# harvardinformatics/IMCoalHMM

Measured on AMD Instinct MI355X. Metric: alignment columns/sec (forward pass), 20-state isolation HMM, higher is better.
Workload: dtype f64

## Files before the change

imcoalhmm_amd/csrc/imcoal_fwd.hip:

```cpp
#include <hip/hip_runtime.h>

#include <algorithm>
#include <array>
#include <cerrno>
#include <climits>
#include <cmath>
#include <cstdint>
#include <cstdio>
#include <cstdlib>
#include <cstring>
#include <list>
#include <atomic>
#include <chrono>
#include <map>
#include <set>
#include <memory>
#include <mutex>
#include <condition_variable>
#include <string>
#include <vector>

#include <sys/stat.h>
#include <unistd.h>

// ... 885 lines not shown
            if (int rc = alloc_symbols(o)) return rc;
            if (int rc = ingest_pump(lk, st, payload, slab, &slabs, fill, [&](int b, uint64_t off, uint64_t len) -> int {
                    const uint32_t columns = (uint32_t)std::min<uint64_t>(4 * len, L - 4 * off);
                    HIP_TRY(hipMemcpyAsync(st.dev[b].get(), st.host[b], (size_t)len, hipMemcpyHostToDevice, g.stream));
                    hipLaunchKernelGGL(k_ing_unpack2, dim3((uint32_t)((len + ING_THREADS - 1) / ING_THREADS)), dim3(ING_THREADS), 0, g.stream,
                                       (const uint8_t *)st.dev[b].get(), columns, o->d_sym + 4 * off * unit, o->wide_raw ? 1 : 0);
                    return IMC_OK;
                }))
                return rc;
            st.release();
            return validate_device_symbols(o->d_sym, (int)unit, (size_t)L, nsym, ">= nsym");
        }
        HIP_TRY(raw.alloc((size_t)payload));
        if (int rc = ingest_pump(lk, st, payload, slab, &slabs, fill, [&](int b, uint64_t off, uint64_t len) -> int {
                HIP_TRY(hipMemcpyAsync(raw.get() + off, st.host[b], (size_t)len, hipMemcpyHostToDevice, g.stream));
                return IMC_OK;
            }))
            return rc;
        st.release();
        const int rc = adopt_device_symbols(o, raw.get(), (int)(h.bits / 8), ">= nsym");
        raw.reset();
        return rc;
    };
    int rc = work();
    if (rc == IMC_OK) rc = finish_device_chunk(lk, o);
    if (rc == IMC_OK) note_ingest(2, payload, slabs, L);
    return ingest_result(rc, o, out);
}

int obs_from_file_device(const char *path, int nsym, imc_obs **out, bool *declined)
{
    FILE *fp = std::fopen(path, "rb");
    if (!fp) return fail(IMC_ERR_IO, std::string("cannot open ") + path + ": " + std::strerror(errno));
    struct Closer { FILE *f; ~Closer() { std::fclose(f); } } closer{fp};
    struct stat sb;
    if (fstat(fileno(fp), &sb) != 0 || !S_ISREG(sb.st_mode)) { *declined = true; return IMC_OK; }
    char head[8];
    const size_t nh = std::fread(head, 1, 8, fp);
    const bool cache = nh == 8 && std::memcmp(head, imc::kCacheMagic, 8) == 0;
    imc::CacheHeader h;
    if (cache) {
        const imc::IoResult hr = imc::read_cache_header(fp, path, nsym, h);
        if (hr.code) return fail(hr.code, hr.msg);
        if (h.bits == 16 && nsym <= imc::kByteAlphabet) { *declined = true; return IMC_OK; }
        if (h.L >= (uint64_t)1 << 31) return fail(IMC_ERR_ARG, "chunk too long (limit 2^31-1 columns per chunk)");
    } else
        std::rewind(fp);
    std::unique_lock<std::mutex> lk(g_mu);
    if (int rc = ensure_ctx()) return rc;
    HIP_TRY(hipSetDevice(g.device));
    return cache ? ingest_cache(lk, fp, h, path, nsym, out) : ingest_text(lk, fp, (uint64_t)sb.st_size, path, nsym, out, declined);
}

int obs_from_pairwise(const char *seq1, const char *seq2, size_t L, imc_obs **out)
{
    std::unique_lock<std::mutex> lk(g_mu);
    if (int rc = ensure_ctx()) return rc;
    HIP_TRY(hipSetDevice(g.device));
    const size_t columns = std::min<size_t>(ingest_slab_bytes() / 2, std::max<size_t>(L, imc::kMinSlabBytes / 2)), half = (columns + 15) & ~(size_t)15;
    IngestStage st;
    if (int rc = st.alloc(2 * half, L > half ? 2 : 1)) return rc;
    imc_obs *o = obs_new(L, 3);
    if (!o) return fail(IMC_ERR_OOM, "host allocation failed");
    uint64_t slabs = 0;
    int rc = alloc_symbols(o);
    if (rc == IMC_OK)
        rc = ingest_pump(lk, st, L, half, &slabs,
                         [&](int b, uint64_t off, uint64_t len) -> int {
                             std::memcpy(st.host[b], seq1 + off, (size_t)len);
                             std::memcpy(st.host[b] + half, seq2 + off, (size_t)len);
                             return IMC_OK;
                         },
                         [&](int b, uint64_t off, uint64_t len) -> int {
                             HIP_TRY(hipMemcpyAsync(st.dev[b].get(), st.host[b], half + (size_t)len, hipMemcpyHostToDevice, g.stream));
                             hipLaunchKernelGGL(k_ing_pairwise, dim3((uint32_t)((len + 4 * ING_THREADS - 1) / (4 * ING_THREADS))), dim3(ING_THREADS), 0, g.stream,
                                                (const uint8_t *)st.dev[b].get(), (const uint8_t *)st.dev[b].get() + half, (uint32_t)len, o->d_sym + off);
                             return IMC_OK;
                         });
    st.release();
    if (rc == IMC_OK) rc = finish_device_chunk(lk, o);
    if (rc == IMC_OK) note_ingest(3, 2 * (uint64_t)L, slabs, L);
    return ingest_result(rc, o, out);
}

int token_level(const imc_obs *obs, int alphabet_limit)
{
    int level = -1;
    if (obs->dict)
        for (int l = 0; l < imc::kNumLevels; ++l)
            if (obs->alphabet[l] <= alphabet_limit && obs->alphabet[l] > obs->nsym && obs->d_tok[l]) level = l;
    return level;
}

int recompress_alphabet(int nsym, std::vector<imc_obs *> &obs, bool on_device)
{
    std::sort(obs.begin(), obs.end(), [](const imc_obs *x, const imc_obs *y) { return x->id < y->id; });
    obs.erase(std::unique(obs.begin(), obs.end()), obs.end());
    const bool wide_raw = nsym > imc::kByteAlphabet;
    const size_t unit = wide_raw ? sizeof(imc::tok_t) : 1;
    PhaseTimer tm;
    size_t total = 0;
    for (imc_obs *o : obs) total += o->L;
    if (total < imc::TrainLimits().train_min) return IMC_OK;
    const size_t share = imc::recompress_share(obs.size(), wide_raw);
    std::vector<std::vector<uint8_t>> raw(obs.size());
    {
        std::lock_guard<std::mutex> lk(g_mu);
        bool same = obs[0]->dict != nullptr;
        for (imc_obs *o : obs) same = same && o->dict == obs[0]->dict;
        if (same && obs[0]->dict->trained_on >= total) return IMC_OK;
        HIP_TRY(hipSetDevice(g.device));
        for (size_t k = 0; k < obs.size(); ++k) {
            raw[k].resize((on_device ? std::min(obs[k]->L, share) : obs[k]->L) * unit);
            HIP_TRY(hipMemcpy(raw[k].data(), obs[k]->d_sym, raw[k].size(), hipMemcpyDeviceToHost));
        }
    }
    std::vector<uint8_t> sample = imc::recompress_sample(raw, share, unit);
    tm.mark();
    const std::shared_ptr<DictDev> nd = make_dictionary(symbols_in(sample, wide_raw), nsym, total);
    std::vector<uint8_t>().swap(sample);
    tm.mark();
    std::vector<imc::EncodedLevels> enc(obs.size());
    const bool zipped = nd->dict.alphabet > nsym;
    if (zipped && !on_device)
        for (size_t k = 0; k < obs.size(); ++k) {
            const HostSymbols sym = symbols_in(raw[k], wide_raw);
            imc::encode_levels(nd->dict, sym.bytes, sym.wide, obs[k]->L, enc[k]);
            std::vector<uint8_t>().swap(raw[k]);
        }
    tm.mark();
    std::unique_lock<std::mutex> lk(g_mu);
    wait_all_idle(lk);
    HIP_TRY(hipSetDevice(g.device));
    HIP_TRY(hipDeviceSynchronize());
    drop_plans_using(obs.data(), obs.size());
    if (!zipped) return IMC_OK;
    if (int rc = publish_dictionary(nsym, nd)) return rc;
    if (on_device) {
        for (imc_obs *o : obs) release_tokens(o);
        if (int rc = device_encode(nd, obs.data(), obs.size())) return rc;
    } else
        for (size_t k = 0; k < obs.size(); ++k) {
            release_tokens(obs[k]);
            if (int rc = install_encoding(obs[k], nd, enc[k])) return rc;
        }
    tm.mark();
    if (PhaseTimer::enabled())
        std::fprintf(stderr, "[imc host] recompress %zu chunks, %zu columns: copy back %.1f ms, train %.1f ms, encode %.1f ms, install %.1f ms (%s encoder)\n",
                     obs.size(), total, tm.ms(0), tm.ms(1), tm.ms(2), tm.ms(3), on_device ? "device" : "host");
    return IMC_OK;
}


using ChainFn = void (*)(const ChainDesc *, int, const uint32_t *, uint32_t, uint32_t, const double *, const int *,
                         const int *, uint32_t, double *, int *, double *, int);

struct KernelChoice : imc::KernelFacts {
    void (*plain)(PropArgs) = nullptr;
    void (*zip)(PropArgs) = nullptr;
    ChainFn chain = nullptr;
    void (*big_table_raw)(BigArgs) = nullptr;
    void (*big_table_level)(BigArgs, const uint16_t *, int) = nullptr;
    void (*big_prop)(BigArgs, const BigBlock *) = nullptr;
    int big_prop_waves = 0;
    void (*big_vec)(BigArgs, const BigBlock *, int, int) = nullptr;
    void (*big_vec_tail)(BigArgs, const BigBlock *, int, int) = nullptr;
    int big_vec_waves = 0;
    void (*zip2)(BigArgs) = nullptr;
    void (*zip3)(BigArgs) = nullptr;
    void (*zip4)(BigArgs) = nullptr;
    void (*zip4w)(BigArgs) = nullptr;
    void (*zip4s)(BigArgs) = nullptr, (*zip4sw)(BigArgs) = nullptr;
    void (*zip4_raw)(BigArgs) = nullptr;
    void (*zip4_level)(BigArgs, int, int) = nullptr;
    void (*zip4_level2)(BigArgs, const int4 *, int, int, const double *) = nullptr;
    void (*zip4_level2_first)(BigArgs, const int4 *, int, int, const double *) = nullptr;
    void (*zip4_level2_split)(BigArgs, const int4 *, int, int, const double *) = nullptr;
    void (*zip4_level2_split_first)(BigArgs, const int4 *, int, int, const double *) = nullptr;
    void (*zip4_level3)(BigArgs, const int4 *, int, int, const double *) = nullptr;
    void (*zip4_level3_first)(BigArgs, const int4 *, int, int, const double *) = nullptr;
    size_t (*zip4_level3_lds)(size_t) = nullptr;
    bool chain_self_emax = false;
    void note_kernels()
    {
        has_zip2 = zip2 != nullptr; has_zip3 = zip3 != nullptr; has_zip4 = zip4 != nullptr; has_zip4s = zip4s != nullptr;
        has_level2 = zip4_level2 != nullptr;
    }
};

template <int R, int G, int MW>
KernelChoice make_kc()
{
    constexpr int NP = R * G;
    KernelChoice k;
    k.R = R; k.G = G; k.NP = NP; k.VPW = 64 / G; k.minw = MW;
    k.zwaves = ZWAVES;
    k.z4_waves = Z2WAVES;
    k.plain = k_propagate<R, G, MW>;
    k.zip = k_zpropagate<R, G>;
    k.zip_lds = &ZipGeom<R, G>::lds_bytes;
    k.chain = k_chain<NP, (NP <= 12 ? 6 : NP <= 24 ? 4 : NP <= 32 ? 3 : NP <= 64 ? 2 : 1)>;
    k.chain_self_emax = true;
    if constexpr (NP % 4 == 0 && NP <= 24) {
        k.zip2 = k_zpropagate2<NP / 4>;
        k.zip2_lds = &Zip2Geom<NP / 4>::lds_bytes;
        k.zip3 = k_zpropagate3<NP / 4>;
        k.zip3_lds = &Zip3Geom<NP / 4>::lds_bytes;
        k.tok_doubles = Zip3Geom<NP / 4>::TOK;
        if constexpr (NP <= 24) {
            k.zip4 = k_zpropagate4<NP / 4, false, true>;
            k.zip4w = k_zpropagate4<NP / 4, true, true>;
            k.zip4s = k_zpropagate4<NP / 4, false, false>;
            k.zip4sw = k_zpropagate4<NP / 4, true, false>;
            k.zip4_raw = k_z4_raw<NP / 4>;
            k.zip4_level = k_z4_level<NP / 4>;
            k.zip4_level2 = k_z4_level2<NP / 4, false>;
            k.zip4_level2_first = k_z4_level2<NP / 4, true>;
            k.zip4_level2_split = k_z4_level2<NP / 4, false, Z4_SPLIT_WAVES>;
            k.zip4_level2_split_first = k_z4_level2<NP / 4, true, Z4_SPLIT_WAVES_FIRST>;
            k.zip4_level3 = k_z4_level3<NP / 4, false>;
            k.zip4_level3_first = k_z4_level3<NP / 4, true>;
            k.zip4_level3_lds = &Z4L3Geom<NP / 4>::lds_bytes;
            k.zip4_lds = &Zip4Geom<NP / 4>::lds_bytes;
            k.zip4_max_hot = &Zip4Geom<NP / 4>::max_hot;
        }
    }
    if constexpr (NP == 28 || NP == 32) {
        k.tok_doubles = Zip3Geom<NP / 4>::TOK;
        k.zip4s = k_zpropagate4<NP / 4, false, false>;
        k.zip4sw = k_zpropagate4<NP / 4, true, false>;
        k.zip4_raw = k_z4_raw<NP / 4>;
        k.zip4_level = k_z4_level<NP / 4>;
        k.zip4_lds = &Zip4Geom<NP / 4>::lds_bytes;
        k.z4_waves = Zip4Shape<NP / 4>::WAVES;
        k.wide_blocked = true;
    }
    k.note_kernels();
    return k;
}

template <int NT, int NSLAB>
KernelChoice make_big()
{
    constexpr bool dealt = NT > 4 && NT % 4 != 0;
    KernelChoice k;
    k.G = NT; k.NP = 16 * NT;
    k.z4_waves = Z2WAVES;
    k.chain = k_chain<16 * NT, 0>;
    k.big_table_raw = k_big_table_raw<NT>;
    k.big_table_level = k_big_table_level<NT>;
    k.big_prop = k_big_propagate<NT, NSLAB>;
    if constexpr (dealt) k.big_prop = k_big_propagate_s<NT, NSLAB>;
    k.big_prop_waves = dealt ? BS_WAVES : NT;
    k.big_vec = k_big_vector<NT, false>;
    k.big_vec_tail = k_big_vector<NT, true>;
    k.big_vec_waves = BigVec<NT>::WAVES;
    k.big_nslab = NSLAB;
    k.big_lds = BigSlab<NT, NSLAB>::bytes;
    return k;
}

KernelChoice kChoices[] = {
    make_kc<4, 1, 2>(), make_kc<4, 2, 2>(), make_kc<4, 3, 2>(), make_kc<4, 4, 2>(), make_kc<4, 5, 2>(),
    make_kc<3, 8, 2>(), make_kc<2, 14, 2>(), make_kc<2, 16, 2>(), make_kc<2, 20, 1>(), make_kc<1, 48, 1>(),
    make_kc<1, 56, 1>(), make_kc<1, 64, 1>(),
    make_big<6, 1>(), make_big<7, 1>(), make_big<8, 2>(), make_big<9, 3>(), make_big<10, 2>(), make_big<12, 3>(), make_big<14, 7>(),
    make_big<16, 8>(),
};
constexpr int IMC_MAX_N = 256;

KernelChoice kMidChoices[] = {make_big<2, 1>(), make_big<3, 1>(), make_big<4, 1>()};

KernelChoice *choose_kernel(int N, bool prefer_gemm)
{
    if (prefer_gemm && N > 24 && N <= 64)
        for (auto &k : kMidChoices)
            if (k.NP >= N) return &k;
    for (auto &k : kChoices)
        if (k.NP >= N) return &k;
    return nullptr;
}


struct Group {
    using Kind = imc::GroupKind;
    Kind kind = Kind::ColumnVector;
    bool is_chain() const { return kind == Kind::GemmChain || kind == Kind::MatVecChain; }
    bool is_blocked() const { return kind == Kind::BlockedLds || kind == Kind::BlockedGlobal; }
    bool global_table() const { return kind == Kind::BlockedGlobal; }

    bool tokens = false;
    int level = -1, A = 0;
    std::shared_ptr<DictDev> dict;
    std::vector<int> chunks;
    uint32_t vec_begin = 0, n_vecs = 0;
    size_t seglen = 0;
    double model_us = 0.0, model_tab_us = 0.0;
    uint64_t vsteps = 0;
    uint64_t stream_len = 0;
    DevBuf<double> d_Ctab;
    DevBuf<int> d_cex;

    struct Chain {
        std::vector<uint32_t> seg_ids, seg_out;
        std::vector<BigBlock> big_blocks;
        DevBuf<BigBlock> d_big_blocks;
        std::vector<std::pair<int, int>> table_runs;
        DevBuf<double> d_Cpack;
        bool rank1 = false;
        std::vector<int> checkpoints;
        std::vector<BigBlock> tail_blocks;
        std::vector<std::pair<uint32_t, uint32_t>> r1_segs;
        DevBuf<BigBlock> d_tail_blocks;
        DevBuf<int> d_r1flag, d_r1at;
        DevBuf<double> d_r1u, d_r1alpha;
    } chain;

    struct Blocked {
        std::vector<Z2Block> blocks;
        DevBuf<Z2Block> d_blocks;
        DevBuf<uint16_t> d_tab_order;
        DevBuf<int> d_tab_lvl;
        std::vector<int> tab_lvl;
        int tab_nlvl = 0;
        DevBuf<int4> d_tab_desc;
        DevBuf<int4> d_tab_desc2;
        std::vector<std::pair<int, int>> tab2;
        DevBuf<int4> d_tab_desc3;
        std::vector<std::pair<int, int>> tab3;
        bool wide_tokens = false;
        bool stream_table = false;
        int n_hot = 0;
        std::vector<uint16_t> hot;
        DevBuf<uint16_t> d_hot;
        imc::PhaseTable phases;
        std::vector<Z2Tail> tails;
        DevBuf<Z2Tail> d_tails;
        DevBuf<double> d_tailX;
        DevBuf<int> d_tailE, d_tail_arrive;
        int tail_stride = 0;
    } blk;
};

struct Level {
    uint32_t n_segs = 0, n_vecs = 0, n_chains = 0;
    DevBuf<uint32_t> d_vec0;
    DevBuf<uint8_t> d_first;
    DevBuf<ChainDesc> d_chains;
    DevBuf<double> d_P;
    DevBuf<int> d_EX, d_EMAX;
};

struct Plan {
    std::vector<uint64_t> key;
// ... 77 lines not shown
    }
    template <class T> void zeroed(DevBuf<T> &d, size_t bytes)
    {
        alloc(d, bytes);
        if (e == hipSuccess) e = hipMemset(d.get(), 0, std::max<size_t>(bytes, 16));
    }
    template <class T, class V> void put(DevBuf<T> &d, const std::vector<V> &h)
    {
        static_assert(sizeof(T) == sizeof(V), "the device buffer holds the host vector's elements");
        alloc(d, h.size() * sizeof(V));
        if (e == hipSuccess && !h.empty()) e = hipMemcpy(d.get(), h.data(), h.size() * sizeof(V), hipMemcpyHostToDevice);
    }
    template <class F> void then(F f)
    {
        if (e == hipSuccess) e = f();
    }
};

struct PlanBuilder {
    const imc_obs *const *chunks = nullptr;
    int n_chunks = 0, N = 0, S = 0, B = 0;
    bool op_mode = false;
    imc::PlanOptions opt;
    KernelChoice *kc = nullptr;
    bool wide = false;
    bool mfma() const { return kc->use3(opt.blocked_variant) || wide; }
    std::unique_ptr<Plan> p;
    std::vector<int> chunk_group;
    std::vector<SegDesc> segs;
    std::vector<uint8_t> seg_first;
    std::vector<uint32_t> chunk_seg;
    std::vector<VecDesc> vecs;
    std::vector<std::vector<std::pair<uint32_t, uint32_t>>> chunk_units;
    std::vector<uint32_t> chunk_unit, unit_vec0;
    std::vector<uint8_t> unit_first;
    struct HostLevel { std::vector<uint32_t> chunk_seg, vec0; std::vector<uint8_t> first; std::vector<ChainDesc> chains; uint32_t n_vecs; };
    std::vector<HostLevel> hl;
    std::vector<int32_t> final_vec;

    void cut_segments()
    {
        chunk_seg.assign(n_chunks + 1, 0);
        for (int f = 0; f < n_chunks; ++f) {
            chunk_seg[f] = (uint32_t)segs.size();
            const Group &gr = p->groups[chunk_group[f]];
            const size_t L = gr.tokens ? chunks[f]->ntok[gr.level] : chunks[f]->L;
            const uint8_t *base = gr.tokens ? chunks[f]->d_tok[gr.level] : chunks[f]->d_sym;
            if (!L) continue;
            const size_t K0 = (L + gr.seglen - 1) / gr.seglen;
            const size_t sl = round_up((L + K0 - 1) / K0, gr.is_blocked() ? Z2GRAN : 16);
            for (size_t off = 0, k = 0; off < L; off += sl, ++k) {
                const bool wide = gr.tokens ? chunks[f]->wide[gr.level] : chunks[f]->wide_raw;
                const bool fst = k == 0 && !op_mode;
                segs.push_back(SegDesc{base + off * (wide ? 2 : 1), (uint32_t)std::min(sl, L - off),
                                       (fst ? SEG_FIRST : 0u) | (wide ? SEG_WIDE : 0u)});
                seg_first.push_back(fst);
            }
        }
        chunk_seg[n_chunks] = (uint32_t)segs.size();
    }

    int make_units()
    {
        chunk_units.assign(n_chunks, {});
        for (int f = 0; f < n_chunks; ++f) {
            const Group &gr = p->groups[chunk_group[f]];
            const uint32_t step = gr.is_blocked() ? (uint32_t)kc->z4_slots() : 1u;
            for (uint32_t sid = chunk_seg[f]; sid < chunk_seg[f + 1]; sid += step)
                chunk_units[f].push_back({sid, std::min(step, chunk_seg[f + 1] - sid)});
        }
        chunk_unit.assign(n_chunks + 1, 0);
        for (int f = 0; f < n_chunks; ++f) chunk_unit[f + 1] = chunk_unit[f] + (uint32_t)chunk_units[f].size();
        unit_vec0.assign(chunk_unit[n_chunks], 0);
        unit_first.assign(chunk_unit[n_chunks], 0);
        for (Group &gr : p->groups) {
            gr.vec_begin = (uint32_t)vecs.size();
            for (int f : gr.chunks) {
                gr.stream_len += gr.tokens ? chunks[f]->ntok[gr.level] : chunks[f]->L;
                for (size_t u = 0; u < chunk_units[f].size(); ++u) {
                    const uint32_t sid = chunk_units[f][u].first, ns = chunk_units[f][u].second;
                    const uint32_t uid = chunk_unit[f] + (uint32_t)u;
                    const bool fst = seg_first[sid] != 0;
                    unit_first[uid] = fst;
                    unit_vec0[uid] = (uint32_t)vecs.size();
                    const int nv = fst ? 1 : N;
                    for (int c = 0; c < nv; ++c) vecs.push_back(VecDesc{sid, (uint32_t)c});
                    if (gr.is_chain()) { gr.chain.seg_ids.push_back(sid); gr.chain.seg_out.push_back(unit_vec0[uid]); }
                    if (gr.is_blocked()) {
                        std::vector<Z2Block> &blocks = gr.blk.blocks;
                        const bool whole = mfma() && fst && ns == 1 && chunk_units[f].size() == 1;
                        if (whole && !blocks.empty() && blocks.back().first == 2 && blocks.back().n < (uint32_t)kc->z4_slots() &&
                            blocks.back().seg0 + blocks.back().n == sid && blocks.back().out_vec0 + blocks.back().n == unit_vec0[uid])
                            ++blocks.back().n;
                        else
                            blocks.push_back(Z2Block{sid, ns, unit_vec0[uid], whole ? 2u : fst ? 1u : 0u});
                    }
                    for (uint32_t q2 = 0; q2 < ns; ++q2)
                        gr.vsteps += (uint64_t)((seg_first[sid + q2] && !gr.is_blocked()) ? 1 : N) * segs[sid + q2].len;
                }
            }
            gr.n_vecs = (uint32_t)vecs.size() - gr.vec_begin;
        }
        if (p->groups.size() == 1 && p->groups[0].is_blocked() && mfma() && !op_mode && n_chunks > 0) {
            Group::Blocked &bl = p->groups[0].blk;
            bool ok = true;
            size_t most = 0;
            for (int f = 0; f < n_chunks; ++f) {
                ok = ok && !chunk_units[f].empty() && chunk_units[f].size() <= (size_t)kc->z4_slots();
                most = std::max(most, chunk_units[f].size());
            }
            if (ok) {
                for (int f : p->groups[0].chunks)
                    for (size_t u = 0; u < chunk_units[f].size(); ++u)
                        bl.tails.push_back(Z2Tail{(uint32_t)f, (uint32_t)u, (uint32_t)chunk_units[f].size(), 0u});
                bl.tail_stride = (int)most;
                if (bl.tails.size() != bl.blocks.size()) bl.tails.clear();
                else
                    for (Z2Block &bk : bl.blocks)
                        if (bk.first == 2) bk.first = 1;
            }
        }
        if (vecs.size() >= (size_t)UINT32_MAX / 2) return fail(IMC_ERR_ARG, "too many vectors in one call");
        p->n_segs = (uint32_t)segs.size();
        p->n_vecs = (uint32_t)vecs.size();
        p->pstride = round_up((size_t)kc->NP + (size_t)kc->NP * kc->NP + (size_t)S * kc->NP, 2);

        return IMC_OK;
    }

    void make_hierarchy()
    {
        hl.assign(1, HostLevel());
        hl[0].chunk_seg = chunk_unit; hl[0].vec0 = unit_vec0; hl[0].first = unit_first; hl[0].n_vecs = p->n_vecs;
        for (;;) {
            const HostLevel &cur = hl.back();
            uint32_t kmax = 0;
            for (int f = 0; f < n_chunks; ++f) kmax = std::max(kmax, cur.chunk_seg[f + 1] - cur.chunk_seg[f]);
            if (kmax <= 1 && hl.size() > 1) break;
            if (kmax == 0) break;
            const uint32_t gsz = kmax <= 16 ? kmax : std::max<uint32_t>(12, (uint32_t)std::ceil(std::cbrt((double)kmax)));
            p->chain_steps += gsz;
            HostLevel nx;
            nx.chunk_seg.assign(n_chunks + 1, 0);
            nx.n_vecs = 0;
            for (int f = 0; f < n_chunks; ++f) {
                nx.chunk_seg[f] = (uint32_t)nx.vec0.size();
                const uint32_t s0 = cur.chunk_seg[f], s1 = cur.chunk_seg[f + 1];
                for (uint32_t rb = s0; rb < s1; rb += gsz) {
                    const uint32_t re = std::min(rb + gsz, s1);
                    const bool fst = rb == s0 && !op_mode;
                    nx.vec0.push_back(nx.n_vecs);
                    nx.first.push_back(fst);
                    const int nvv = fst ? 1 : N;
                    for (int c = 0; c < nvv; ++c) nx.chains.push_back(ChainDesc{rb, re, (uint32_t)c, nx.n_vecs + c, fst ? 1u : 0u, 0u});
                    nx.n_vecs += nvv;
                }
            }
            nx.chunk_seg[n_chunks] = (uint32_t)nx.vec0.size();
            const bool done = kmax <= gsz;
            hl.push_back(std::move(nx));
            if (done) break;
        }
        final_vec.assign(std::max(n_chunks, 1), -1);
        bool all_from_chains = hl.size() > 1 && !op_mode && n_chunks > 0;
        for (int f = 0; f < n_chunks; ++f) {
            const HostLevel &last = hl.back();
            if (last.chunk_seg[f + 1] > last.chunk_seg[f]) final_vec[f] = (int32_t)last.vec0[last.chunk_seg[f]];
            else all_from_chains = false;
        }
        p->finish_fused = false;
        if (all_from_chains) {
            HostLevel &last = hl.back();
            std::vector<char> seen((size_t)n_chunks, 0);
            for (ChainDesc &cd : last.chains)
                for (int f = 0; f < n_chunks; ++f)
                    if (cd.first && final_vec[f] == (int32_t)cd.out_vec) { cd.chunk1 = (uint32_t)f + 1; seen[f] = 1; }
            p->finish_fused = std::all_of(seen.begin(), seen.end(), [](char c) { return c != 0; });
            if (!p->finish_fused)
                for (ChainDesc &cd : last.chains) cd.chunk1 = 0;
        }

    }

    int upload(Plan **out)
    {
        while (g_plans.size() >= MAX_PLANS) {
            auto victim = g_plans.end();
            for (auto it = g_plans.begin(); it != g_plans.end(); ++it)
                if (!(*it)->busy) victim = it;
            if (victim == g_plans.end()) break;
            g_plans.erase(victim);
        }

        Plan *q = p.get();
        DevUpload u;
        u.put(q->d_segs, segs);
        u.put(q->d_vecs, vecs);
        u.put(q->d_final_vec, final_vec);
        q->levels.resize(hl.size());
        for (size_t l = 0; l < hl.size(); ++l) {
            Level &lv = q->levels[l];
            lv.n_segs = (uint32_t)hl[l].vec0.size();
            lv.n_vecs = hl[l].n_vecs;
            lv.n_chains = (uint32_t)hl[l].chains.size();
            const size_t nv = std::max<size_t>(lv.n_vecs, 1), ns = std::max<size_t>(lv.n_segs, 1);
            u.put(lv.d_vec0, hl[l].vec0);
            u.put(lv.d_first, hl[l].first);
            u.put(lv.d_chains, hl[l].chains);
            u.zeroed(lv.d_P, (size_t)B * nv * kc->NP * 8);
            u.zeroed(lv.d_EX, (size_t)B * nv * 4);
            u.zeroed(lv.d_EMAX, (size_t)B * ns * 4);
        }
        for (Group &gr : q->groups) {
            Group::Blocked &bl = gr.blk;
            Group::Chain &ch = gr.chain;
            if (gr.is_blocked()) u.put(bl.d_blocks, bl.blocks);
            if (!bl.tails.empty()) {
                const size_t slots = (size_t)B * n_chunks * bl.tail_stride;
                u.put(bl.d_tails, bl.tails);
                u.alloc(bl.d_tailX, slots * kc->tok_doubles * 8);
                u.alloc(bl.d_tailE, slots * 128);
                u.zeroed(bl.d_tail_arrive, (size_t)B * n_chunks * 4);
            }
            if (gr.global_table()) {
                std::vector<uint64_t> cnt((size_t)gr.A, 0);
                for (int f : gr.chunks)
                    for (size_t z = 0; z < chunks[f]->tok_count[gr.level].size() && z < cnt.size(); ++z) cnt[z] += chunks[f]->tok_count[gr.level][z];
                const std::vector<uint16_t> ids = imc::hot_order(cnt);
                const double tables = (double)B * (gr.A + 1) * kc->tok_doubles * 8.0;
                bl.stream_table = wide || imc::z4_streamed(opt, tables, B);
                bl.n_hot = bl.stream_table ? 0 : std::min(gr.A, kc->zip4_max_hot(gr.A, LDS_BUDGET));
                bl.hot.assign(ids.begin(), ids.begin() + bl.n_hot);
                bl.phases = imc::xcd_phases(B, (int)bl.blocks.size());
                u.put(bl.d_hot, bl.hot);
                u.alloc(gr.d_Ctab, (size_t)B * (gr.A + 1) * kc->tok_doubles * 8);
                u.alloc(gr.d_cex, (size_t)B * (gr.A + 1) * 4 + 16);
            }
            if (gr.is_blocked() && gr.tokens) {
                const DictDev &dd = *gr.dict;
                const imc::DepthOrder o = imc::depth_order_below(dd.order, dd.depth, gr.A);
                bl.tab_nlvl = o.nlvl;
                bl.tab_lvl = o.lvl;
                u.put(bl.d_tab_order, o.order);
                u.put(bl.d_tab_lvl, o.lvl);
                if (gr.global_table()) {
                    const std::vector<imc::Desc4> desc = imc::level_descriptors(dd.dict, o);
                    const imc::TableSchedule s2 = imc::pairs_schedule(dd.dict, dd.depth, o, S);
                    const imc::TableSchedule s3 = imc::triples_schedule(dd.dict, dd.depth, o, S, gr.A);
                    bl.tab2 = s2.launches;
                    bl.tab3 = s3.launches;
                    u.put(bl.d_tab_desc, desc);
                    if (!s2.desc.empty()) u.put(bl.d_tab_desc2, s2.desc);
                    if (!s3.desc.empty()) u.put(bl.d_tab_desc3, s3.desc);
                }
            }
            if (!gr.is_chain()) continue;
            const size_t np2 = (size_t)kc->NP * kc->NP;
            if (gr.tokens) ch.table_runs = imc::depth_runs_below(gr.dict->order, gr.dict->depth, gr.A);
            ch.big_blocks = imc::deal_slabs<BigBlock>(ch.seg_ids, ch.seg_out, seg_first, kc->big_nslab);
            u.put(ch.d_big_blocks, ch.big_blocks);
            u.alloc(gr.d_Ctab, (size_t)B * gr.A * np2 * 8);
            if ((gr.kind == Group::Kind::MatVecChain || ch.rank1) && N < kc->NP && g.pack_table)
                u.alloc(ch.d_Cpack, (size_t)B * gr.A * N * (size_t)(N + (N & 1)) * 8);
            u.alloc(gr.d_cex, (size_t)B * gr.A * 4 + 16);
            if (ch.rank1) {
                ch.tail_blocks = imc::tail_list<BigBlock>(ch.seg_ids, ch.seg_out);
                for (uint32_t id : ch.seg_ids)
                    if (!seg_first[id]) ch.r1_segs.push_back({id, segs[id].len});
                const size_t nrec = (size_t)B * segs.size();
                u.put(ch.d_tail_blocks, ch.tail_blocks);
                u.zeroed(ch.d_r1flag, nrec * 4);
                u.zeroed(ch.d_r1at, nrec * 4);
                u.alloc(ch.d_r1u, nrec * kc->NP * 8);
                u.alloc(ch.d_r1alpha, nrec * kc->NP * 8);
            }
        }
        u.alloc(q->d_params, (size_t)B * q->pstride * 8);
        u.alloc(q->d_out, (size_t)B * std::max(n_chunks, 1) * 8);
        for (int k = 0; k < 2; ++k) {
            u.then([&] { return hipHostMalloc((void **)&q->h_params[k], (size_t)B * q->pstride * 8, hipHostMallocMapped); });
            u.then([&] { return hipHostGetDevicePointer((void **)&q->h_params_dev[k], q->h_params[k], 0); });
            u.then([&] { return hipEventCreateWithFlags(&q->ev_params[k], hipEventDisableTiming); });
        }
        u.then([&] { return hipHostMalloc((void **)&q->h_out, (size_t)B * std::max(n_chunks, 1) * 8, hipHostMallocMapped); });
        u.then([&] { return hipHostGetDevicePointer((void **)&q->h_out_dev, q->h_out, 0); });
        if (u.e != hipSuccess)
            return fail(u.e == hipErrorOutOfMemory ? IMC_ERR_OOM : IMC_ERR_HIP,
                        std::string("plan allocation: ") + hipGetErrorString(u.e));
        g_plans.push_front(std::move(p));
        *out = q;
        return IMC_OK;
    }
};

void gather_facts(const imc_obs *const *chunks, int n_chunks, std::vector<imc::ChunkFacts> &cf, std::vector<imc::DictFacts> &df,
                  std::vector<std::shared_ptr<DictDev>> &dict_of)
{
    cf.resize(n_chunks);
    for (int f = 0; f < n_chunks; ++f) {
        const imc_obs *o = chunks[f];
        imc::ChunkFacts &c = cf[f];
        c.L = o->L; c.nsym = o->nsym; c.wide_raw = o->wide_raw;
        if (o->dict) {
            c.dict = (int)(std::find(dict_of.begin(), dict_of.end(), o->dict) - dict_of.begin());
            if (c.dict == (int)dict_of.size()) { dict_of.push_back(o->dict); df.push_back(imc::DictFacts{&o->dict->depth}); }
        }
        for (int l = 0; l < imc::kNumLevels; ++l)
// ... 274 lines not shown
    return IMC_OK;
}


BigArgs Launch::blocked_args(const Group &gr)
{
    BigArgs ba = common_args(p, gr);
    ba.blocks = gr.blk.d_blocks.get();
    ba.n_group_segs = (uint32_t)gr.blk.blocks.size();
    ba.tab_order = gr.blk.d_tab_order.get(); ba.tab_lvl = gr.blk.d_tab_lvl.get(); ba.tab_nlvl = gr.blk.tab_nlvl;
    ba.hot = gr.blk.d_hot.get(); ba.n_hot = gr.blk.n_hot; ba.tab_desc = gr.blk.d_tab_desc.get();
    if (gr.blk.d_tails && (g.fuse_tail == 2 || (g.fuse_tail == 1 && gr.blk.tail_stride <= 4)) && allow_tail && (p->kc->use3(g.blocked_variant) || p->wide)) {
        ba.tail = gr.blk.d_tails.get(); ba.tailX = gr.blk.d_tailX.get(); ba.tailE = gr.blk.d_tailE.get(); ba.tail_arrive = gr.blk.d_tail_arrive.get();
        ba.tail_out = out; ba.tail_stride = gr.blk.tail_stride;
        tail_used = true;
    }
    return ba;
}

int Launch::z4_table(const Group &gr, const BigArgs &ba)
{
    const double *const staged = p->h_params_dev[p->slot], *const none = nullptr;
    bool head = fuse_head;
    if (!fuse_head) {
        hipLaunchKernelGGL(kc->zip4_raw, dim3((unsigned)p->S + 1, (unsigned)B), dim3(256), 0, stream, ba);
        HIP_TRY(hipGetLastError());
    }
    if (g.table_pairs && (g.table_triples == 1 || (g.table_triples < 0 && kc->NP <= 12)) && gr.blk.d_tab_desc3 && kc->zip4_level3) {
        if (int rc = allow_lds_budget(kc->zip4_level3)) return rc;
        if (int rc = allow_lds_budget(kc->zip4_level3_first)) return rc;
        for (const auto &lc : gr.blk.tab3) {
            const dim3 grid((unsigned)(lc.second + Z4L3_WAVES - 1) / Z4L3_WAVES, (unsigned)B);
            if (head)
                hipLaunchKernelGGL(kc->zip4_level3_first, grid, dim3(Z4L3_WAVES * 64), kc->zip4_level3_lds(p->pstride), stream, ba,
                                   (const int4 *)gr.blk.d_tab_desc3.get(), lc.first, lc.second, staged);
            else
                hipLaunchKernelGGL(kc->zip4_level3, grid, dim3(Z4L3_WAVES * 64), kc->zip4_level3_lds(0), stream, ba,
                                   (const int4 *)gr.blk.d_tab_desc3.get(), lc.first, lc.second, none);
            head = false;
            HIP_TRY(hipGetLastError());
        }
    } else if (g.table_pairs && gr.blk.d_tab_desc2 && kc->zip4_level2) {
        const size_t split_max = g.table_split_max >= 0 ? (size_t)g.table_split_max : (size_t)4 * g.cus;
        for (const auto &lc : gr.blk.tab2) {
            if (g.table_split && (size_t)lc.second * B <= split_max) {
                if (head)
                    hipLaunchKernelGGL(kc->zip4_level2_split_first, dim3((unsigned)(lc.second + Z4_SPLIT_WAVES_FIRST - 1) / Z4_SPLIT_WAVES_FIRST, (unsigned)B),
                                       dim3(Z4_SPLIT_WAVES_FIRST * 64), p->pstride * 8, stream, ba,
                                       (const int4 *)gr.blk.d_tab_desc2.get(), lc.first, lc.second, staged);
                else
                    hipLaunchKernelGGL(kc->zip4_level2_split, dim3((unsigned)(lc.second + Z4_SPLIT_WAVES - 1) / Z4_SPLIT_WAVES, (unsigned)B),
                                       dim3(Z4_SPLIT_WAVES * 64), 0, stream, ba,
                                       (const int4 *)gr.blk.d_tab_desc2.get(), lc.first, lc.second, none);
                split_used = true;
            } else if (head)
                hipLaunchKernelGGL(kc->zip4_level2_first, dim3((unsigned)(lc.second + 3) / 4, (unsigned)B), dim3(64),
                                   p->pstride * 8, stream, ba,
                                   (const int4 *)gr.blk.d_tab_desc2.get(), lc.first, lc.second, staged);
            else
                hipLaunchKernelGGL(kc->zip4_level2, dim3((unsigned)(lc.second + 3) / 4, (unsigned)B), dim3(64), 0, stream, ba,
                                   (const int4 *)gr.blk.d_tab_desc2.get(), lc.first, lc.second, none);
            head = false;
            HIP_TRY(hipGetLastError());
        }
    } else
        for (int d = 0; d < gr.blk.tab_nlvl; ++d) {
            const int first = gr.blk.tab_lvl[d], count = gr.blk.tab_lvl[d + 1] - first;
            hipLaunchKernelGGL(kc->zip4_level, dim3((unsigned)(count + 3) / 4, (unsigned)B), dim3(64), 0, stream, ba, first, count);
            HIP_TRY(hipGetLastError());
        }
    return IMC_OK;
}

int Launch::zip4(const Group &gr)
{
    BigArgs ba = blocked_args(gr);
    if (int rc = z4_table(gr, ba)) return rc;
    void (*scan)(BigArgs) = gr.blk.stream_table ? (gr.blk.wide_tokens ? kc->zip4sw : kc->zip4s) : (gr.blk.wide_tokens ? kc->zip4w : kc->zip4);
    if (int rc = allow_lds_budget(scan)) return rc;
    if (int rc = mark_a()) return rc;
    dim3 scan_grid(ba.n_group_segs, (unsigned)B);
    if (g.xcd_affine && B > 1) {
        const imc::PhaseTable &t = gr.blk.phases;
        ba.n_phases = t.n_phases;
        for (int k = 0; k < t.n_phases; ++k) { ba.ph_begin[k] = t.ph_begin[k]; ba.ph_first[k] = t.ph_first[k]; ba.ph_sets[k] = t.ph_sets[k]; }
        scan_grid = dim3((unsigned)t.grid);
    }
    hipLaunchKernelGGL(scan, scan_grid, dim3(kc->z4_waves * 64), kc->zip4_lds(gr.A, gr.blk.n_hot), stream, ba);
    note(std::string("k_zpropagate4<") + std::to_string(kc->NP / 4) + (gr.blk.wide_tokens ? ",16" : "") + (gr.blk.stream_table ? ",streamed>" : ">") + stream_tag(gr));
    account(gr);
    HIP_TRY(hipGetLastError());
    return IMC_OK;
}

int Launch::zip32(const Group &gr)
{
    BigArgs ba = blocked_args(gr);
    const bool v3 = kc->use3(g.blocked_variant);
    void (*scan)(BigArgs) = v3 ? kc->zip3 : kc->zip2;
    if (int rc = allow_lds_budget(scan)) return rc;
    size_t lds3 = kc->blocked_lds(gr.A, g.blocked_variant);
    if (direct_params) { ba.params_src = p->h_params_dev[p->slot]; lds3 = ((lds3 + 15) & ~(size_t)15) + p->pstride * 8; }
    hipLaunchKernelGGL(scan, dim3(ba.n_group_segs, (unsigned)p->B), dim3(Z2WAVES * 64), lds3, stream, ba);
    note(std::string(v3 ? "k_zpropagate3<" : "k_zpropagate2<") + std::to_string(kc->NP / 4) + ">" + stream_tag(gr));
    account(gr);
    HIP_TRY(hipGetLastError());
    return IMC_OK;
}


int Launch::zpropagate(const Group &gr)
{
    const size_t lds = kc->zip_lds(gr.A);
    if (int rc = allow_lds_budget(kc->zip)) return rc;
    const uint32_t vpb = (uint32_t)(ZWAVES * kc->VPW);
    dim3 grid((gr.n_vecs + vpb - 1) / vpb, (unsigned)p->B);
    hipLaunchKernelGGL(kc->zip, grid, dim3(ZWAVES * 64), lds, stream, prop_args(p, gr));
    note("k_zpropagate<" + std::to_string(kc->R) + "," + std::to_string(kc->G) + ">" + stream_tag(gr));
    account(gr);
    HIP_TRY(hipGetLastError());
    return IMC_OK;
}

int Launch::propagate(const Group &gr)
{
    const uint32_t vpb = (uint32_t)(WPB * kc->VPW);
    dim3 grid((gr.n_vecs + vpb - 1) / vpb, (unsigned)p->B);
    const size_t lds = ((size_t)WPB * kc->VPW * kc->NP + (size_t)p->S * kc->NP) * 8;
    if (lds > LDS_BUDGET) return fail(IMC_ERR_ARG, "emission table (S x N) too large for LDS");
    if (lds > 48 * 1024)
        if (int rc = allow_lds_budget(kc->plain)) return rc;
    hipLaunchKernelGGL(kc->plain, grid, dim3(WPB * 64), lds, stream, prop_args(p, gr));
    note("k_propagate<" + std::to_string(kc->R) + "," + std::to_string(kc->G) + ">" + stream_tag(gr));
    account(gr);
    HIP_TRY(hipGetLastError());
    return IMC_OK;
}


int Launch::stitch() const
{
    const int N = p->N, NP = kc->NP;
    for (size_t l = 0; l + 1 < p->levels.size(); ++l) {
        const Level &in = p->levels[l], &ot = p->levels[l + 1];
        if (!in.n_segs || !ot.n_chains) continue;
        if (!kc->chain_self_emax) {
            hipLaunchKernelGGL(k_emax, dim3((in.n_segs + 255) / 256, (unsigned)B), dim3(256), 0, stream,
                               in.d_vec0.get(), in.d_first.get(), in.n_segs, in.n_vecs, N, in.d_EX.get(), in.d_EMAX.get());
            HIP_TRY(hipGetLastError());
        }
        const int threads = (int)round_up((size_t)NP, 64);
        const bool last_level = l + 2 == p->levels.size();
        hipLaunchKernelGGL(kc->chain, dim3(ot.n_chains, (unsigned)B), dim3(threads), 0, stream,
                           ot.d_chains.get(), N, in.d_vec0.get(), in.n_segs, in.n_vecs, in.d_P.get(), in.d_EX.get(), in.d_EMAX.get(),
                           ot.n_vecs, ot.d_P.get(), ot.d_EX.get(), (last_level && p->finish_fused) ? out : (double *)nullptr, p->n_chunks);
        HIP_TRY(hipGetLastError());
    }
    if (p->n_chunks && !p->finish_fused) {
        const Level &last = p->levels.back();
        hipLaunchKernelGGL(k_finish, dim3((p->n_chunks + 63) / 64, (unsigned)B), dim3(64), 0, stream,
                           p->d_final_vec.get(), p->n_chunks, N, NP, last.n_vecs, last.d_P.get(), last.d_EX.get(), out);
        HIP_TRY(hipGetLastError());
    }
    return IMC_OK;
}

int enqueue(Plan *p, hipStream_t stream, double *out, bool allow_tail = true)
{
    hipStreamCaptureStatus cap = hipStreamCaptureStatusNone;
    (void)hipStreamIsCapturing(stream, &cap);
    if (cap == hipStreamCaptureStatusNone && p->have_last && p->last_stream != stream)
        HIP_TRY(hipStreamWaitEvent(stream, p->ev_params[p->last_slot], 0));
    Launch L{p, stream, out, allow_tail};
    if (int rc = L.fetch_params()) return rc;

    uint64_t *lp = p->lp;
    lp[0] = p->n_segs; lp[1] = p->n_vecs; lp[2] = lp[3] = lp[4] = lp[5] = lp[6] = lp[7] = 0;
    L.prof = g.profile && p->n_vecs;
    if (L.prof) { HIP_TRY(hipEventCreate(&L.ev.a)); HIP_TRY(hipEventCreate(&L.ev.b)); HIP_TRY(hipEventCreate(&L.ev.c)); }
    p->kernels.clear();
    for (const Group &gr : p->groups) {
        if (!gr.n_vecs) continue;
        if (!gr.global_table())
            if (int rc = L.mark_a()) return rc;
        int rc = IMC_OK;
        switch (gr.kind) {
        case Group::Kind::ColumnVector: rc = L.propagate(gr); break;
        case Group::Kind::TokenVector: rc = L.zpropagate(gr); break;
        case Group::Kind::BlockedLds: rc = L.zip32(gr); break;
        case Group::Kind::BlockedGlobal: rc = L.zip4(gr); break;
        case Group::Kind::GemmChain: rc = L.gemm_chain(gr); break;
        case Group::Kind::MatVecChain: rc = L.matvec_chain(gr); break;
        }
        if (rc) return rc;
    }
    if (int rc = L.mark_a()) return rc;
    if (L.prof) HIP_TRY(hipEventRecord(L.ev.b, stream));
    if (L.split_used) L.note("table-split");
    if (L.tail_used) L.note("fused-tail");
    if (!L.tail_used)
        if (int rc = L.stitch()) return rc;
    if (L.prof) {
        HIP_TRY(hipEventRecord(L.ev.c, stream));
        g.events.push_back(L.ev);
    }
    if (cap == hipStreamCaptureStatusNone) {
        HIP_TRY(hipEventRecord(p->ev_params[p->slot], stream));
        p->ev_used[p->slot] = true;
        p->last_stream = stream;
        p->last_slot = p->slot;
        p->have_last = true;
    }
    return IMC_OK;
}

void collect_rank1_stats(Plan *p)
{
    g.r1_checked = g.r1_collapsed = 0;
    for (Group &gr : p->groups) {
        if (!gr.chain.rank1 || gr.chain.r1_segs.empty() || gr.chain.checkpoints.empty()) continue;
        std::vector<int> flags((size_t)p->B * p->n_segs);
        if (hipMemcpy(flags.data(), gr.chain.d_r1flag.get(), flags.size() * 4, hipMemcpyDeviceToHost) != hipSuccess) continue;
        for (int b = 0; b < p->B; ++b)
            for (const auto &sl : gr.chain.r1_segs) {
                if ((int)sl.second <= gr.chain.checkpoints[0]) continue;
                ++g.r1_checked;
                g.r1_collapsed += flags[(size_t)b * p->n_segs + sl.first] ? 1 : 0;
            }
        if (getenv("IMC_DEBUG_R1")) {
            std::vector<int> at((size_t)p->B * p->n_segs);
            if (hipMemcpy(at.data(), gr.chain.d_r1at.get(), at.size() * 4, hipMemcpyDeviceToHost) != hipSuccess) continue;
            std::map<int, int> hist;
            for (const auto &sl : gr.chain.r1_segs) hist[flags[sl.first] ? at[sl.first] : -1]++;
            fprintf(stderr, "[imc] rank-one hand-off: segment length %zu tokens, checkpoints", (size_t)gr.seglen);
            for (int c : gr.chain.checkpoints) fprintf(stderr, " %d", c);
            fprintf(stderr, "\n[imc]   certified at (tokens: segments)");
            for (auto &kv : hist) fprintf(stderr, " %d:%d", kv.first, kv.second);
            fprintf(stderr, "\n");
        }
    }
}

constexpr uint64_t OUT_SENTINEL = 0x7ff8dead5e471e15ull;

hipError_t wait_results(hipStream_t st, const double *h_out, size_t n)
{
    const volatile uint64_t *v = reinterpret_cast<const volatile uint64_t *>(h_out);
    const auto t0 = std::chrono::steady_clock::now();
    size_t k = 0;
    for (unsigned spin = 0;; ++spin) {
        while (k < n && v[k] != OUT_SENTINEL) ++k;
        if (k == n) { std::atomic_thread_fence(std::memory_order_acquire); return hipSuccess; }
        if ((spin & 63) == 63 && std::chrono::steady_clock::now() - t0 > std::chrono::milliseconds(2)) return hipStreamSynchronize(st);
    }
}

int run_batch(const imc_obs *const *chunks, int n_chunks, int B, int N, int S, const double *pis, const double *Ts,
              const double *Es, double *out_sum, double *out_per_chunk)
{
    std::unique_lock<std::mutex> lk(g_mu);
    static const bool dbg_host = std::getenv("IMC_DEBUG_HOST") != nullptr;
    auto now = [] { return std::chrono::steady_clock::now(); };
    const auto h0 = now();
    if (int rc = ensure_ctx()) return rc;
    if (int rc = check_args(chunks, n_chunks, B, N, S, pis, Ts, Es)) return rc;
    HIP_TRY(hipSetDevice(g.device));
    Plan *p = nullptr;
    for (;;) {
        if (int rc = build_plan(chunks, n_chunks, N, S, B, false, &p)) return rc;
        if (!p->busy) break;
        g_cv.wait(lk);
    }
    struct Busy {
        Plan *p;
        explicit Busy(Plan *q) : p(q) { p->busy = true; }
        ~Busy() { p->busy = false; g_cv.notify_all(); }
    } busy(p);
    const auto h1 = now();
    if (int rc = stage_params(p, pis, Ts, Es, g.use_graphs)) return rc;
    const size_t n_out = (size_t)B * n_chunks;
    for (size_t k = 0; k < n_out; ++k) reinterpret_cast<volatile uint64_t *>(p->h_out)[k] = OUT_SENTINEL;
    std::atomic_thread_fence(std::memory_order_release);
    const auto h2 = now();
    const bool use_graph = !g.profile && g.use_graphs && p->calls >= 1;
    if (use_graph && !p->graph) {
        hipGraph_t gr = nullptr;
        HIP_TRY(hipStreamBeginCapture(g.stream, hipStreamCaptureModeThreadLocal));
        const int rc = enqueue(p, g.stream, p->h_out_dev);
        const hipError_t ec = hipStreamEndCapture(g.stream, &gr);
        if (rc) { if (gr) (void)hipGraphDestroy(gr); return rc; }
        if (ec != hipSuccess) return fail(IMC_ERR_HIP, std::string("hipStreamEndCapture: ") + hipGetErrorString(ec));
        const hipError_t ei = hipGraphInstantiate(&p->graph, gr, nullptr, nullptr, 0);
        (void)hipGraphDestroy(gr);
        if (ei != hipSuccess) { p->graph = nullptr; return fail(IMC_ERR_HIP, std::string("hipGraphInstantiate: ") + hipGetErrorString(ei)); }
    }
    if (use_graph) HIP_TRY(hipGraphLaunch(p->graph, g.stream));
    else if (int rc = enqueue(p, g.stream, p->h_out_dev)) return rc;
    ++p->calls;
    publish_last(p);
    const auto h3 = now();
    const hipStream_t st = g.stream;
    lk.unlock();
    const hipError_t ew = n_out ? wait_results(st, p->h_out, n_out) : hipStreamSynchronize(st);
    lk.lock();
    HIP_TRY(ew);
    const auto h4 = now();
    collect_rank1_stats(p);
// ... 880 lines not shown
```

imcoalhmm_amd/csrc/kernels_stitch.hpp:

```cpp
#pragma once
#include "kernels_plain.hpp"

struct ChainDesc {
    uint32_t seg_begin, seg_end;
    uint32_t c;
    uint32_t out_vec;
    uint32_t first;
    uint32_t chunk1;
};

__global__ void k_emax(const uint32_t *seg_vec0, const uint8_t *seg_first, uint32_t n_segs, uint32_t n_vecs, int N,
                       const int *EX, int *EMAX)
{
    const uint32_t s = blockIdx.x * blockDim.x + threadIdx.x;
    const int b = blockIdx.y;
    if (s >= n_segs) return;
    const int *e = EX + (size_t)b * n_vecs + seg_vec0[s];
    int m = e[0];
    if (!seg_first[s])
        for (int c = 1; c < N; ++c) m = max(m, e[c]);
    EMAX[(size_t)b * n_segs + s] = m;
}

template <int NP, int D>
__global__ __launch_bounds__(((NP + 63) / 64) * 64) void k_chain(
    const ChainDesc *chains, int N,
    const uint32_t *in_vec0, uint32_t in_n_segs, uint32_t in_n_vecs, const double *Pin, const int *EXin, const int *EMin,
    uint32_t out_n_vecs, double *Pout, int *EXout, double *fin_out, int n_chunks)
{
    __shared__ __attribute__((aligned(16))) double w[2][NP];
    constexpr bool ONE_WAVE = NP <= 64;
    auto sync = [&]() { if (ONE_WAVE) wave_fence(); else __syncthreads(); };
    const ChainDesc cd = chains[blockIdx.x];
    const int b = blockIdx.y, i = threadIdx.x;
    const double *Pb = Pin + (size_t)b * in_n_vecs * NP;
    const int *EXb = EXin + (size_t)b * in_n_vecs;
    const int *EMb = EMin + (size_t)b * in_n_segs;
    const bool mine = i < N;
    const int ii = mine ? i : 0;

    double a;
    int etot;
    uint32_t k0 = cd.seg_begin;
    if (cd.first) {
        const uint32_t v = in_vec0[k0];
        a = mine ? Pb[(size_t)v * NP + i] : 0.0;
        etot = EXb[v];
        ++k0;
    } else {
        a = (i == (int)cd.c) ? 1.0 : 0.0;
        etot = 0;
    }
    const int nsteps = (int)cd.seg_end - (int)k0;
    const uint32_t vbase = nsteps > 0 ? in_vec0[k0] : 0u;

    if constexpr (D == 0) {
        int buf = 0;
        for (int t = 0; t < nsteps; ++t) {
            const size_t v0 = (size_t)vbase + (size_t)t * N;
            const int em = EMb[k0 + t];
            if (mine) w[buf][i] = ldexp(a, EXb[v0 + ii] - em);
            else if (i < NP) w[buf][i] = 0.0;
            sync();
            const double2 *row = reinterpret_cast<const double2 *>(Pb + (v0 + ii) * NP);
            const double2 *wv = reinterpret_cast<const double2 *>(&w[buf][0]);
            double acc0 = 0.0, acc1 = 0.0, s0 = 0.0, s1 = 0.0;
#pragma unroll 4
            for (int m = 0; m < NP / 2; ++m) {
                const double2 wc = wv[m], pc = row[m];
                acc0 = fma(pc.x, wc.x, acc0);
                acc1 = fma(pc.y, wc.y, acc1);
                s0 += wc.x;
                s1 += wc.y;
            }
            const double sm = s0 + s1;
            int e = 0;
            (void)frexp(sm, &e);
            e = (sm > 0.0 && sm < INFINITY) ? e : 0;
            a = mine ? ldexp(acc0 + acc1, -e) : 0.0;
            etot += em + e;
            buf ^= 1;
        }
    } else {
    double2 pk[D > 0 ? D : 1][NP / 2];
    int exr[D > 0 ? D : 1];
    auto fetch = [&](int t, int slot) {
        const size_t v0 = (size_t)vbase + (size_t)t * N;
        exr[slot] = EXb[v0 + ii];
        const double2 *row = reinterpret_cast<const double2 *>(Pb + (v0 + ii) * NP);
#pragma unroll
        for (int m = 0; m < NP / 2; ++m) pk[slot][m] = row[m];
    };
#pragma unroll
    for (int s = 0; s < D; ++s)
        if (s < nsteps) fetch(s, s);
    int buf = 0;
    for (int t0 = 0; t0 < nsteps; t0 += D) {
#pragma unroll
        for (int s = 0; s < D; ++s) {
            const int t = t0 + s;
            if (t < nsteps) {
                const int em = wave_max_i32_dpp(exr[s]);
                if (mine) w[buf][i] = ldexp(a, exr[s] - em);
                else if (i < NP) w[buf][i] = 0.0;
                double2 cur[NP / 2];
#pragma unroll
                for (int m = 0; m < NP / 2; ++m) cur[m] = pk[s][m];
                if (t + D < nsteps) fetch(t + D, s);
                sync();
                double acc0 = 0.0, acc1 = 0.0, s0 = 0.0, s1 = 0.0;
                const double2 *wv = reinterpret_cast<const double2 *>(&w[buf][0]);
#pragma unroll
                for (int m = 0; m < NP / 2; ++m) {
                    const double2 wc = wv[m];
                    acc0 = fma(cur[m].x, wc.x, acc0);
                    acc1 = fma(cur[m].y, wc.y, acc1);
                    s0 += wc.x;
                    s1 += wc.y;
                }
                const double sm = s0 + s1;
                int e = 0;
                (void)frexp(sm, &e);
                e = (sm > 0.0 && sm < INFINITY) ? e : 0;
                a = mine ? ldexp(acc0 + acc1, -e) : 0.0;
                etot += em + e;
                buf ^= 1;
            }
        }
    }
    }
    sync();
    if (i < NP) w[0][i] = mine ? a : 0.0;
    sync();
    double tot = 0.0;
    for (int c = 0; c < N; ++c) tot += w[0][c];
    int e = 0;
    (void)frexp(tot, &e);
    e = (tot > 0.0 && tot < INFINITY) ? e : 0;
    const size_t gv = (size_t)b * out_n_vecs + cd.out_vec;
    if (mine) {
        double *dst = cd.first ? Pout + gv * NP + i : Pout + (gv - cd.c) * NP + (size_t)i * NP + cd.c;
        *dst = ldexp(a, -e);
    }
    if (i == 0) {
        EXout[gv] = etot + e;
        if (fin_out && cd.chunk1)
            fin_out[(size_t)b * n_chunks + (cd.chunk1 - 1)] = (double)(etot + e) * 0.693147180559945309417232121458 + log(ldexp(tot, -e));
    }
}

__global__ void k_finish(const int32_t *final_vec, int n_chunks, int N, int NP, uint32_t n_vecs, const double *P,
                         const int *EX, double *out)
{
    const int f = blockIdx.x * blockDim.x + threadIdx.x;
    const int b = blockIdx.y;
    if (f >= n_chunks) return;
    const int32_t v = final_vec[f];
    double r = 0.0;
    if (v >= 0) {
        const double *p = P + ((size_t)b * n_vecs + v) * NP;
        double tot = 0.0;
        for (int c = 0; c < N; ++c) tot += p[c];
        r = (double)EX[(size_t)b * n_vecs + v] * 0.693147180559945309417232121458 + log(tot);
    }
    out[(size_t)b * n_chunks + f] = r;
}

__global__ void k_export(const int32_t *final_vec, int n_chunks, int N, int NP, uint32_t n_vecs, const double *P,
                         const int *EX, int op, double *out_state, int *out_exp)
{
    const int f = blockIdx.x, b = blockIdx.y;
    const int32_t v = final_vec[f];
    if (v < 0) return;
    const double *src = P + ((size_t)b * n_vecs + v) * NP;
    const int *ex = EX + (size_t)b * n_vecs + v;
    if (op) {
        double *dst = out_state + ((size_t)b * n_chunks + f) * N * N;
        int *de = out_exp + ((size_t)b * n_chunks + f) * N;
        for (int idx = threadIdx.x; idx < N * N; idx += blockDim.x) {
            const int i = idx / N, c = idx - i * N;
            dst[idx] = src[(size_t)i * NP + c];
        }
        for (int c = threadIdx.x; c < N; c += blockDim.x) de[c] = ex[c];
    } else {
        double *dst = out_state + ((size_t)b * n_chunks + f) * N;
        for (int i = threadIdx.x; i < N; i += blockDim.x) dst[i] = src[i];
        if (threadIdx.x == 0) out_exp[(size_t)b * n_chunks + f] = ex[0];
    }
}

__global__ void k_stage_params(const double2 *__restrict__ src, double2 *__restrict__ dst, unsigned n2)
{
    const unsigned i = blockIdx.x * blockDim.x + threadIdx.x;
    if (i < n2) dst[i] = src[i];
}

__global__ void k_sum_chunks(const double *per_chunk, int n_chunks, int B, double *partial)
{
    const int b = blockIdx.x * blockDim.x + threadIdx.x;
    if (b >= B) return;
    double t = 0.0;
    for (int f = 0; f < n_chunks; ++f) t += per_chunk[(size_t)b * n_chunks + f];
    partial[b] = t;
}
```

Baseline: 394.1 billion.

## Precompute chain vector bases on host and restructure stitch prefetch ring

The chain kernel no longer reads in_vec0 on the device to find its first and base vectors. The host now computes these indices and stores them in two new ChainDesc fields, which removes a dependent global load before the prefetch can start. The step loop is restructured into a steady-state loop without per-step bounds checks, followed by an unrolled tail, with compiler barriers added to keep the prefetch ordering. The ring depth is fixed at 2 for all state counts (previously 4 for 20 states), which lowers register pressure but hides less load latency.

```diff
diff --git a/imcoalhmm_amd/csrc/imcoal_fwd.hip b/imcoalhmm_amd/csrc/imcoal_fwd.hip
--- a/imcoalhmm_amd/csrc/imcoal_fwd.hip
+++ b/imcoalhmm_amd/csrc/imcoal_fwd.hip
@@ -1061,7 +1061,7 @@
 }
 
 
-using ChainFn = void (*)(const ChainDesc *, int, const uint32_t *, uint32_t, uint32_t, const double *, const int *,
+using ChainFn = void (*)(const ChainDesc *, int, uint32_t, uint32_t, const double *, const int *,
                          const int *, uint32_t, double *, int *, double *, int);
 
 struct KernelChoice : imc::KernelFacts {
@@ -1108,7 +1108,7 @@
     k.plain = k_propagate<R, G, MW>;
     k.zip = k_zpropagate<R, G>;
     k.zip_lds = &ZipGeom<R, G>::lds_bytes;
-    k.chain = k_chain<NP, (NP <= 12 ? 6 : NP <= 24 ? 4 : NP <= 32 ? 3 : NP <= 64 ? 2 : 1)>;
+    k.chain = k_chain<NP, chain_ring_depth(NP)>;
     k.chain_self_emax = true;
     if constexpr (NP % 4 == 0 && NP <= 24) {
         k.zip2 = k_zpropagate2<NP / 4>;
@@ -1492,7 +1492,10 @@
                     nx.vec0.push_back(nx.n_vecs);
                     nx.first.push_back(fst);
                     const int nvv = fst ? 1 : N;
-                    for (int c = 0; c < nvv; ++c) nx.chains.push_back(ChainDesc{rb, re, (uint32_t)c, nx.n_vecs + c, fst ? 1u : 0u, 0u});
+                    const uint32_t op0 = rb + (fst ? 1u : 0u);
+                    const uint32_t vec_first = fst ? cur.vec0[rb] : 0u, vbase = op0 < re ? cur.vec0[op0] : 0u;
+                    for (int c = 0; c < nvv; ++c)
+                        nx.chains.push_back(ChainDesc{rb, re, (uint32_t)c, nx.n_vecs + c, fst ? 1u : 0u, 0u, vec_first, vbase});
                     nx.n_vecs += nvv;
                 }
             }
@@ -2073,7 +2076,7 @@
         const int threads = (int)round_up((size_t)NP, 64);
         const bool last_level = l + 2 == p->levels.size();
         hipLaunchKernelGGL(kc->chain, dim3(ot.n_chains, (unsigned)B), dim3(threads), 0, stream,
-                           ot.d_chains.get(), N, in.d_vec0.get(), in.n_segs, in.n_vecs, in.d_P.get(), in.d_EX.get(), in.d_EMAX.get(),
+                           ot.d_chains.get(), N, in.n_segs, in.n_vecs, in.d_P.get(), in.d_EX.get(), in.d_EMAX.get(),
                            ot.n_vecs, ot.d_P.get(), ot.d_EX.get(), (last_level && p->finish_fused) ? out : (double *)nullptr, p->n_chunks);
         HIP_TRY(hipGetLastError());
     }
diff --git a/imcoalhmm_amd/csrc/kernels_stitch.hpp b/imcoalhmm_amd/csrc/kernels_stitch.hpp
--- a/imcoalhmm_amd/csrc/kernels_stitch.hpp
+++ b/imcoalhmm_amd/csrc/kernels_stitch.hpp
@@ -7,6 +7,8 @@
     uint32_t out_vec;
     uint32_t first;
     uint32_t chunk1;
+    uint32_t vec_first;
+    uint32_t vbase;
 };
 
 __global__ void k_emax(const uint32_t *seg_vec0, const uint8_t *seg_first, uint32_t n_segs, uint32_t n_vecs, int N,
@@ -25,7 +27,7 @@
 template <int NP, int D>
 __global__ __launch_bounds__(((NP + 63) / 64) * 64) void k_chain(
     const ChainDesc *chains, int N,
-    const uint32_t *in_vec0, uint32_t in_n_segs, uint32_t in_n_vecs, const double *Pin, const int *EXin, const int *EMin,
+    uint32_t in_n_segs, uint32_t in_n_vecs, const double *Pin, const int *EXin, const int *EMin,
     uint32_t out_n_vecs, double *Pout, int *EXout, double *fin_out, int n_chunks)
 {
     __shared__ __attribute__((aligned(16))) double w[2][NP];
@@ -43,7 +45,7 @@
     int etot;
     uint32_t k0 = cd.seg_begin;
     if (cd.first) {
-        const uint32_t v = in_vec0[k0];
+        const uint32_t v = cd.vec_first;
         a = mine ? Pb[(size_t)v * NP + i] : 0.0;
         etot = EXb[v];
         ++k0;
@@ -52,7 +54,7 @@
         etot = 0;
     }
     const int nsteps = (int)cd.seg_end - (int)k0;
-    const uint32_t vbase = nsteps > 0 ? in_vec0[k0] : 0u;
+    const uint32_t vbase = cd.vbase;
 
     if constexpr (D == 0) {
         int buf = 0;
@@ -82,50 +84,66 @@
             buf ^= 1;
         }
     } else {
-    double2 pk[D > 0 ? D : 1][NP / 2];
-    int exr[D > 0 ? D : 1];
+    typedef double v2d __attribute__((ext_vector_type(2)));
+    v2d pk[D][NP / 2];
+    int exr[D];
     auto fetch = [&](int t, int slot) {
         const size_t v0 = (size_t)vbase + (size_t)t * N;
         exr[slot] = EXb[v0 + ii];
-        const double2 *row = reinterpret_cast<const double2 *>(Pb + (v0 + ii) * NP);
+        const v2d *row = reinterpret_cast<const v2d *>(Pb + (v0 + ii) * NP);
 #pragma unroll
         for (int m = 0; m < NP / 2; ++m) pk[slot][m] = row[m];
     };
-#pragma unroll
-    for (int s = 0; s < D; ++s)
-        if (s < nsteps) fetch(s, s);
     int buf = 0;
-    for (int t0 = 0; t0 < nsteps; t0 += D) {
+    auto step = [&](int s) {
+        int ex = exr[s];
+        asm volatile("" : "+v"(ex));
+        const int em = wave_max_i32_dpp(ex);
+        if (mine) w[buf][i] = ldexp(a, ex - em);
+        else if (i < NP) w[buf][i] = 0.0;
+        sync();
+        double acc0 = 0.0, acc1 = 0.0, s0 = 0.0, s1 = 0.0;
+        const double2 *wv = reinterpret_cast<const double2 *>(&w[buf][0]);
+#pragma unroll
+        for (int m = 0; m < NP / 2; ++m) {
+            const double2 wc = wv[m];
+            acc0 = fma(pk[s][m].x, wc.x, acc0);
+            acc1 = fma(pk[s][m].y, wc.y, acc1);
+            s0 += wc.x;
+            s1 += wc.y;
+        }
+        const double sm = s0 + s1;
+        int e = 0;
+        (void)frexp(sm, &e);
+        e = (sm > 0.0 && sm < INFINITY) ? e : 0;
+        a = mine ? ldexp(acc0 + acc1, -e) : 0.0;
+        etot += em + e;
+        buf ^= 1;
+    };
+    auto refill = [&](int t, int slot) {
+        asm volatile("" : "+v"(a) : : "memory");
+        fetch(t, slot);
+    };
+    if (nsteps > 0) {
+        const int last = nsteps - 1;
 #pragma unroll
         for (int s = 0; s < D; ++s) {
-            const int t = t0 + s;
-            if (t < nsteps) {
-                const int em = wave_max_i32_dpp(exr[s]);
-                if (mine) w[buf][i] = ldexp(a, exr[s] - em);
-                else if (i < NP) w[buf][i] = 0.0;
-                double2 cur[NP / 2];
-#pragma unroll
-                for (int m = 0; m < NP / 2; ++m) cur[m] = pk[s][m];
-                if (t + D < nsteps) fetch(t + D, s);
-                sync();
-                double acc0 = 0.0, acc1 = 0.0, s0 = 0.0, s1 = 0.0;
-                const double2 *wv = reinterpret_cast<const double2 *>(&w[buf][0]);
-#pragma unroll
-                for (int m = 0; m < NP / 2; ++m) {
-                    const double2 wc = wv[m];
-                    acc0 = fma(cur[m].x, wc.x, acc0);
-                    acc1 = fma(cur[m].y, wc.y, acc1);
-                    s0 += wc.x;
-                    s1 += wc.y;
-                }
-                const double sm = s0 + s1;
-                int e = 0;
-                (void)frexp(sm, &e);
-                e = (sm > 0.0 && sm < INFINITY) ? e : 0;
-                a = mine ? ldexp(acc0 + acc1, -e) : 0.0;
-                etot += em + e;
-                buf ^= 1;
+            fetch(min(s, last), s);
+            asm volatile("" : : : "memory");
+        }
+        int t0 = 0;
+        for (; t0 + 2 * D <= nsteps; t0 += D) {
+#pragma unroll
+            for (int s = 0; s < D; ++s) {
+                step(s);
+                refill(t0 + s + D, s);
             }
+        }
+#pragma unroll
+        for (int j = 0; j < 2 * D - 1; ++j) {
+            step(j % D);
+            if (t0 + j + 1 >= nsteps) break;
+            if (j < D - 1) refill(min(t0 + j + D, last), j);
         }
     }
     }
@@ -149,6 +167,8 @@
     }
 }
 
+constexpr int chain_ring_depth(int ) { return 2; }
+
 __global__ void k_finish(const int32_t *final_vec, int n_chunks, int N, int NP, uint32_t n_vecs, const double *P,
                          const int *EX, double *out)
 {
```

After: 396.8 billion (median of 5 runs). About the same (+0.7%).
